# m-schuetz/SimLOD

Measured on NVIDIA H100. Metric: Mpoints/sec octree insertion (16B XYZRGBA), higher is better.
Workload: dtype u32+f32

## Files before the change

### simlod_b200/csrc/construct.cu

```cuda
#include <cooperative_groups.h>
#include <stdint.h>
#include "../../include/simlod_abi.h"
#include "fpmath.cuh"

namespace cg = cooperative_groups;

typedef SimlodPoint Point;
typedef SimlodChunk Chunk;
typedef SimlodNode Node;
typedef SimlodStats Stats;
typedef SimlodUniforms Uniforms;
typedef SimlodHeapHeader Heap;
struct CudaPrint;

#include "construct_layout.cuh"

enum : uint32_t {
    ERR_SPILL_OVERFLOW  = 1u << 0,
    ERR_VOXEL_OVERFLOW  = 1u << 1,
    ERR_DIR_OVERFLOW    = 1u << 2,
    ERR_NODE_OVERFLOW   = 1u << 3,
    ERR_QUEUE_OVERFLOW  = 1u << 4,
    ERR_SPILLNODE_OVERFLOW = 1u << 5,
    ERR_ROW_OVERFLOW    = 1u << 6,
// ... 105 lines not shown
__device__ __forceinline__ bool nested(const Coords& q) {
    return ((((q.pX >> 8) ^ q.X) | ((q.pY >> 8) ^ q.Y) | ((q.pZ >> 8) ^ q.Z)) & 0xfffffu) == 0;
}
__device__ __forceinline__ uint32_t childIndexAt(const Coords& q, uint32_t level) {
    uint32_t sh = SIMLOD_MAX_DEPTH - 1 - level;
    return (((q.X >> sh) & 1u) << 2) | (((q.Y >> sh) & 1u) << 1) | ((q.Z >> sh) & 1u);
}
__device__ __forceinline__ uint32_t cellAt(const Coords& q, uint32_t level) {
    uint32_t sh = SIMLOD_MAX_DEPTH + 1 - level;
    uint32_t cx = (q.pX >> sh) & 127u, cy = (q.pY >> sh) & 127u, cz = (q.pZ >> sh) & 127u;
    return cx | (cy << 7) | (cz << 14);
}

__shared__ uint32_t sh_allocTarget;
__shared__ uint32_t sh_allocSeen;

__device__ __forceinline__ void waitAllocThread(const Ctx& c) {
    const uint32_t target = sh_allocTarget;
    if (target == 0 || *(volatile uint32_t*)&sh_allocSeen) return;
    while ((int32_t)(ldAcquire(&c.ctl()->allocDone) - target) < 0) __nanosleep(64);
    *(volatile uint32_t*)&sh_allocSeen = 1;
}
__device__ __forceinline__ void waitAllocBlock(const Ctx& c) {
    if (sh_allocTarget != 0) {
        if (threadIdx.x == 0) waitAllocThread(c);
        __syncthreads();
    }
}

#ifndef SIMLOD_VOXTAB_SIZE
#define SIMLOD_VOXTAB_SIZE 64
#endif
constexpr uint32_t VOXTAB_SIZE = SIMLOD_VOXTAB_SIZE;
static_assert((VOXTAB_SIZE & (VOXTAB_SIZE - 1)) == 0 && VOXTAB_SIZE <= 128, "table size: a power of two, two tables are flushed by one 256-thread block, the index is packed into 7 bits");
constexpr uint32_t VOXTAB_EMPTY = 0xffffffffu;
__shared__ uint32_t sh_tabKey[VOXTAB_SIZE];
__shared__ uint32_t sh_tabCount[VOXTAB_SIZE];
__shared__ uint32_t sh_tabBase[VOXTAB_SIZE];
__shared__ uint32_t sh_cursor;
__shared__ uint32_t sh_passStart;

__device__ __forceinline__ uint32_t tabHash(uint32_t key) { return (key * 0x9E3779B1u) >> 26; }
__device__ __forceinline__ uint32_t tabFind(const uint32_t* keys, uint32_t key) {
    uint32_t h = tabHash(key);
#pragma unroll 1
    for (uint32_t probe = 0; probe < VOXTAB_SIZE; probe++) {
        uint32_t s = (h + probe) & (VOXTAB_SIZE - 1);
        uint32_t k = keys[s];
        if (k == key) return s;
        if (k == VOXTAB_EMPTY) break;
    }
    return VOXTAB_EMPTY;
}
__device__ __forceinline__ uint32_t tabInsert(uint32_t* keys, uint32_t key) {
    uint32_t h = tabHash(key);
#pragma unroll 1
    for (uint32_t probe = 0; probe < VOXTAB_SIZE; probe++) {
        uint32_t s = (h + probe) & (VOXTAB_SIZE - 1);
        uint32_t k = atomicCAS(&keys[s], VOXTAB_EMPTY, key);
        if (k == VOXTAB_EMPTY || k == key) return s;
    }
    return VOXTAB_EMPTY;
}

__device__ __forceinline__ void voxelPassBegin(const Ctx& c, const Batch& b, bool firstPassOfBatch) {
    if (threadIdx.x < VOXTAB_SIZE) { sh_tabKey[threadIdx.x] = VOXTAB_EMPTY; sh_tabCount[threadIdx.x] = 0; }
    if (threadIdx.x == 0) { sh_cursor = firstPassOfBatch ? 0u : c.blockCursor(b.parity)[blockIdx.x]; sh_passStart = sh_cursor; }
}

__device__ __noinline__ void recordVoxelShared(uint32_t node, uint32_t cell, uint32_t color) {
    const Ctx c;
    const Batch& b = sh_batch;
    waitAllocThread(c);
    Node* nd = &c.nodes()[node];
    uint32_t vslot = atomicAdd(&nd->numVoxels, 1u);
    if (vslot == ldv(&nd->numVoxelsStored)) { uint32_t d = atomicAdd(&b.bc->numDirtyVox, 1u); c.dirtyVox(b.parity)[d] = node; }
    atomicAdd(&b.bc->voxelsCreated, 1u);
    uint32_t e = atomicAdd(&b.bc->numBacklog, 1u);
    if (e < scratch::VOXEL_SHARED) {
        uint64_t at = scratch::VOXEL_CAP - scratch::VOXEL_SHARED + e;
        c.vkey(b.parity)[at] = (uint64_t)cell | ((uint64_t)node << 21) | ((uint64_t)vslot << 41);
        c.vcolor(b.parity)[at] = color;
    } else {
        atomicOr(&c.ctl()->errorFlags, ERR_VOXEL_OVERFLOW);
    }
}

__device__ __forceinline__ void recordVoxel(const Ctx& c, const Batch& b, uint32_t node, uint32_t cell, uint32_t color) {
    const uint32_t active = __activemask();
    const uint32_t leader = __ffs(active) - 1u;
    const uint32_t node0 = __shfl_sync(active, node, leader);
    if (__all_sync(active, node == node0)) {
        const uint32_t n = __popc(active), mine = __popc(active & lanemaskLt());
        uint32_t slot = 0, idx0 = 0, rank0 = 0, fit = 0;
        if (laneId() == leader) {
            slot = tabInsert(sh_tabKey, node0);
            if (slot != VOXTAB_EMPTY) {
                idx0 = atomicAdd(&sh_cursor, n);
                fit = idx0 < c.segCap() ? min(n, c.segCap() - idx0) : 0u;
                if (fit) rank0 = atomicAdd(&sh_tabCount[slot], fit);
            }
        }
        slot = __shfl_sync(active, slot, leader); idx0 = __shfl_sync(active, idx0, leader); rank0 = __shfl_sync(active, rank0, leader); fit = __shfl_sync(active, fit, leader);
        if (mine >= fit) { recordVoxelShared(node, cell, color); return; }
        const uint64_t at = (uint64_t)blockIdx.x * c.segCap() + idx0 + mine;
        c.vkey(b.parity)[at] = (uint64_t)cell | ((uint64_t)slot << 21) | ((uint64_t)(rank0 + mine) << 41);
        c.vcolor(b.parity)[at] = color;
        return;
    }
    uint32_t slot = tabInsert(sh_tabKey, node);
    if (slot == VOXTAB_EMPTY) { recordVoxelShared(node, cell, color); return; }
    uint32_t idx = atomicAdd(&sh_cursor, 1u);
    if (idx >= c.segCap()) { recordVoxelShared(node, cell, color); return; }
    uint32_t rank = atomicAdd(&sh_tabCount[slot], 1u);
    uint64_t at = (uint64_t)blockIdx.x * c.segCap() + idx;
    c.vkey(b.parity)[at] = (uint64_t)cell | ((uint64_t)slot << 21) | ((uint64_t)rank << 41);
    c.vcolor(b.parity)[at] = color;
}

__device__ __forceinline__ void voxelFlushEntry(const Ctx& c, const Batch& b, uint32_t entry) {
    uint32_t node = sh_tabKey[entry], cnt = sh_tabCount[entry];
    if (node != VOXTAB_EMPTY && cnt > 0) {
        Node* nd = &c.nodes()[node];
        uint32_t base = atomicAdd(&nd->numVoxels, cnt);
        if (base == ldv(&nd->numVoxelsStored)) {
            uint32_t d = atomicAdd(&b.bc->numDirtyVox, 1u);
            c.dirtyVox(b.parity)[d] = node;
        }
        sh_tabBase[entry] = base;
    }
}
__device__ __forceinline__ void voxelFlushPatch(const Ctx& c, const Batch& b, bool freshPass) {
    const uint32_t endIdx = min(sh_cursor, c.segCap());
    uint64_t* vkey = c.vkey(b.parity);
    for (uint32_t e = sh_passStart + threadIdx.x; e < endIdx; e += blockDim.x) {
        uint64_t at = (uint64_t)blockIdx.x * c.segCap() + e;
        uint64_t k = vkey[at];
        uint32_t slot = (uint32_t)(k >> 21) & (VOXTAB_SIZE - 1);
        uint32_t rank = (uint32_t)(k >> 41);
        vkey[at] = (k & 0x1fffffull) | ((uint64_t)sh_tabKey[slot] << 21) | ((uint64_t)(sh_tabBase[slot] + rank) << 41);
    }
    if (threadIdx.x == 0) {
        c.blockCursor(b.parity)[blockIdx.x] = endIdx;
        if (endIdx > sh_passStart) {
            atomicAdd(&b.bc->voxelsCreated, endIdx - sh_passStart);
            atomicAdd(reinterpret_cast<unsigned long long*>(&c.ctl()->voxelsTotal), (unsigned long long)(endIdx - sh_passStart));
            atomicAdd(reinterpret_cast<unsigned long long*>(&c.ctl()->voxelsByPass[freshPass ? 0 : 1]), (unsigned long long)(endIdx - sh_passStart));
        }
    }
}

constexpr uint32_t PROVISIONAL = 0x80000000u;
static_assert(scratch::ITEM_CAP < (1u << 24), "block-local ranks must fit 24 bits");
__shared__ uint32_t sh_leafKey[VOXTAB_SIZE];
__shared__ uint32_t sh_leafCount[VOXTAB_SIZE];
__shared__ uint32_t sh_leafBase[VOXTAB_SIZE];
__shared__ uint8_t  sh_leafLevel[VOXTAB_SIZE];
__device__ __forceinline__ uint32_t finalSlot(uint32_t sl) { return (sl & PROVISIONAL) ? sh_leafBase[(sl >> 24) & 127u] + (sl & 0xffffffu) : sl; }
constexpr uint32_t RUNSLOT_CAP = 2048;
__shared__ uint32_t sh_runSlot[RUNSLOT_CAP];
constexpr uint32_t LIST_CAP = 2048;
__shared__ uint32_t sh_listCount;
__shared__ uint32_t sh_listMode;
__shared__ uint32_t sh_blockLegacy;
__shared__ uint8_t  sh_entrySplit[VOXTAB_SIZE];
constexpr uint32_t WL_SPLIT_SHIFT = 22;
constexpr uint32_t WL_ITEM_MASK = (1u << WL_SPLIT_SHIFT) - 1u;
static_assert(scratch::ITEM_CAP <= (1u << WL_SPLIT_SHIFT), "worklist entries keep the item in 22 bits");
__shared__ uint32_t sh_splitNodes[64];
__shared__ SpillInfo sh_splitInfo[64];
__shared__ uint32_t sh_splitGranule[65];
__shared__ uint32_t sh_wlCount, sh_wlBase, sh_wlFill;
__shared__ uint32_t sh_roundLegacy, sh_roundListed;
__device__ __forceinline__ uint32_t blockExclusiveScan(uint32_t v, uint32_t& total) {
    __shared__ uint32_t sh_warpSum[8];
    __shared__ uint32_t sh_total;
    const uint32_t lane = laneId(), warp = threadIdx.x >> 5;
    uint32_t incl = v;
#pragma unroll
    for (int o = 1; o < 32; o <<= 1) { uint32_t t = __shfl_up_sync(0xffffffffu, incl, o); if (lane >= (uint32_t)o) incl += t; }
    __syncthreads();
    if (lane == 31) sh_warpSum[warp] = incl;
    __syncthreads();
    if (threadIdx.x == 0) { uint32_t run = 0; for (int w = 0; w < 8; w++) { uint32_t t = sh_warpSum[w]; sh_warpSum[w] = run; run += t; } sh_total = run; }
    __syncthreads();
    total = sh_total;
    return sh_warpSum[warp] + incl - v;
}

constexpr uint32_t BLOOM_WORDS = 8;
constexpr uint32_t AFFECTED_CAP = 1024;
__shared__ uint32_t sh_runBloom[BLOOM_WORDS];
__shared__ uint32_t sh_affected[AFFECTED_CAP];
__shared__ uint32_t sh_numAffected;
__device__ __forceinline__ uint32_t bloomHash(uint32_t node) { return (node * 0x9E3779B1u) >> 24; }
__device__ __forceinline__ void bloomAdd(uint32_t* bloom, uint32_t node) { uint32_t h = bloomHash(node); atomicOr(&bloom[h >> 5], 1u << (h & 31u)); }

struct Rewalk { uint32_t perRun, runItems, total, spilledBefore; bool listed; };
__device__ __forceinline__ Rewalk rewalkSlice(uint32_t numBatch, uint32_t numSpilled, uint32_t spilledBefore) {
    Rewalk r;
    r.perRun = ((numBatch + gridDim.x - 1) / gridDim.x + 31u) & ~31u;
    r.listed = gridDim.x <= AFFECTED_CAP;
    r.runItems = (r.listed ? sh_numAffected : gridDim.x) * r.perRun;
    r.total = r.runItems + numSpilled;
    r.spilledBefore = spilledBefore;
    return r;
}
__device__ __forceinline__ uint32_t rewalkFirstGranule() { return ((threadIdx.x >> 5) * gridDim.x + blockIdx.x) * 32u; }
__device__ __forceinline__ uint32_t rewalkGranuleStride() { return gridDim.x * blockDim.x; }
__device__ __forceinline__ uint32_t rewalkItem(const Rewalk& r, uint32_t u, uint32_t& run) {
    run = 0xffffffffu;
    if (u >= r.runItems) return (uint32_t)scratch::MAX_BATCH + (u - r.runItems);
    const uint32_t k = u / r.perRun;
    run = r.listed ? sh_affected[k] : k;
    return run * r.perRun + (u - k * r.perRun);
}

__device__ __noinline__ uint32_t countGlobal(uint32_t node, uint32_t level, uint32_t cnt) {
    const Ctx c;
    const Batch& b = sh_batch;
    waitAllocThread(c);
    Node* leaf = &c.nodes()[node];
    uint32_t old = atomicAdd(&leaf->counter, cnt);
    uint32_t stored = ldv(&leaf->numPoints);
    if (old == stored) {
        uint32_t d = atomicAdd(&b.bc->numDirtyLeaves, 1u);
        c.dirtyLeaves(b.parity)[d] = node;
    }
    if (old + cnt > SIMLOD_MAX_POINTS_PER_NODE && atomicCAS(&c.splitState()[node], 0u, 1u) == 0u) {
        uint32_t err = 0;
        const uint32_t childBase = atomicAdd(&c.stats()->numNodes, 8u);
        if ((uint64_t)childBase + 8 > scratch::NODE_CAP) { err = ERR_NODE_OVERFLOW; atomicSub(&c.stats()->numNodes, 8u); }
        uint32_t base = 0;
        if (!err && stored) {
            base = atomicAdd(&b.bc->numSpilled, stored);
            if ((uint64_t)base + stored > scratch::SPILL_CAP) { err = ERR_SPILL_OVERFLOW; atomicSub(&b.bc->numSpilled, stored); atomicSub(&c.stats()->numNodes, 8u); }
        }
        uint32_t s = 0;
        if (!err) {
            s = atomicAdd(&b.bc->numSpillTotal, 1u);
            if (s >= scratch::SPILLNODE_CAP) {
                err = ERR_SPILLNODE_OVERFLOW; atomicSub(&b.bc->numSpillTotal, 1u);
                if (stored) atomicSub(&b.bc->numSpilled, stored);
                atomicSub(&c.stats()->numNodes, 8u);
            }
        }
        if (err) {
            atomicOr(&c.ctl()->errorFlags, err);
            atomicAdd(&c.ctl()->events[3], 1u);
            atomicExch(&c.splitState()[node], 0u);
        } else {
            SpillInfo info;
            info.node = node;
            info.stored = stored;
            info.level = level;
            info.row = c.leafRow()[node];
            info.base = base;
            info.childBase = childBase;
            uint64_t g = c.gridPtr()[node];
            if (g == 0) g = (uint64_t)(c.heapBytes() + atomicAdd(reinterpret_cast<unsigned long long*>(&c.heap()->offset), (unsigned long long)SIMLOD_GRID_STRIDE));
            info.grid = g;
            c.spill()[s] = info;
        }
    }
    return old;
}

struct LeafCache { uint32_t leaf, parent; uint64_t key; };
__device__ __forceinline__ uint64_t leafKey(const Coords& q, uint32_t level) {
    const uint32_t sh = SIMLOD_MAX_DEPTH - level;
    return (uint64_t)((q.X & 0xfffffu) >> sh) | ((uint64_t)((q.Y & 0xfffffu) >> sh) << 20) | ((uint64_t)((q.Z & 0xfffffu) >> sh) << 40);
}

template <bool MIXED_RUNS = false>
__device__ __forceinline__ uint32_t countInto(const Ctx& c, const Batch& b, bool valid, uint32_t node, uint32_t level, uint32_t* bloom, bool forceGlobal) {
    const uint32_t lane = laneId();
    uint32_t slot = 0;
    const uint32_t vmask = __ballot_sync(0xffffffffu, valid);
    if (valid) {
        uint32_t peers = __match_any_sync(vmask, node);
        uint32_t leader = __ffs(peers) - 1;
        uint32_t cnt = __popc(peers);
        uint32_t r = 0;
        if (lane == leader) {
            uint32_t t = forceGlobal ? VOXTAB_EMPTY : tabInsert(sh_leafKey, node);
            if (t != VOXTAB_EMPTY) { r = atomicAdd(&sh_leafCount[t], cnt) | PROVISIONAL | (t << 24); sh_leafLevel[t] = (uint8_t)level; }
            else                 { r = countGlobal(node, level, cnt); sh_blockLegacy = 1; if (!forceGlobal) atomicAdd(&c.ctl()->events[2], 1u); }
            if (bloom) bloomAdd(bloom, node);
        }
        r = __shfl_sync(peers, r, leader);
        slot = r + __popc(peers & lanemaskLt());
        if (MIXED_RUNS) {
            const uint64_t leaderBloom = __shfl_sync(peers, (uint64_t)(uintptr_t)bloom, leader);
            if (bloom && (uint64_t)(uintptr_t)bloom != leaderBloom) bloomAdd(bloom, node);
        }
    }
    return slot;
}

template <bool UNCACHED_GRID, bool DEDUP>
__device__ __forceinline__ void sampleUp(const Ctx& c, const Batch& b, const Coords& q, uint32_t color, uint32_t sNode, uint32_t sLevel, uint32_t stopLevel) {
    const uint32_t lane = laneId();
    const bool exhaustive = !nested(q);
    if (exhaustive) atomicOr(&c.ctl()->errorFlags, ERR_FAR_POINT);
    uint32_t pending = 0;
    uint32_t old0 = 0, old1 = 0, old2 = 0, key0 = 0, key1 = 0, key2 = 0, cel0 = 0, cel1 = 0, cel2 = 0;
    auto settle = [&]() {
        if (pending > 0 && (old0 & (1u << (cel0 & 31u))) == 0) recordVoxel(c, b, key0, cel0, color);
        if (pending > 1 && (old1 & (1u << (cel1 & 31u))) == 0) recordVoxel(c, b, key1, cel1, color);
        if (pending > 2 && (old2 & (1u << (cel2 & 31u))) == 0) recordVoxel(c, b, key2, cel2, color);
        pending = 0;
    };
    const uint64_t* gridPtr = c.gridPtr();
    for (;;) {
        uint64_t g = gridPtr[sNode];
        bool goUp = exhaustive;
        if (g != 0) {
            uint32_t cell = cellAt(q, sLevel);
            uint32_t* word = reinterpret_cast<uint32_t*>(g) + (cell >> 5);
            uint32_t bit = 1u << (cell & 31u);
            uint32_t seen = UNCACHED_GRID ? ldcg(word) : *word;
            if ((seen & bit) == 0) {
                bool mine = true;
                if (DEDUP) {
                    uint32_t active = __activemask();
                    uint32_t peers = __match_any_sync(active, (uint64_t)(uintptr_t)word * 32ull + (cell & 31u));
                    mine = lane == (uint32_t)__ffs(peers) - 1u;
                }
                if (mine) {
                    if (pending == 3) settle();
                    uint32_t old = atomicOr(word, bit);
                    if (pending == 0) { old0 = old; key0 = sNode; cel0 = cell; }
                    else if (pending == 1) { old1 = old; key1 = sNode; cel1 = cell; }
                    else { old2 = old; key2 = sNode; cel2 = cell; }
                    pending++;
                    goUp = true;
                }
            }
        }
        if (!goUp || sLevel <= stopLevel) break;
        sNode = c.parentOf()[sNode];
        sLevel--;
    }
    settle();
}

template <bool SAMPLE, bool COUNT, bool UNCACHED_GRID, bool DEDUP>
__device__ __forceinline__ void walk(const Ctx& c, const Batch& b, LeafCache& cache, bool valid, uint4 pt, uint32_t node, uint32_t level,
                                     uint32_t stopLevel, uint32_t* bloom, bool forceGlobal, uint32_t& leafPacked, uint32_t& slot) {
    Coords q = quantize(c, pt);
    uint32_t parent = VOXTAB_EMPTY;
    if (valid) {
        if (cache.leaf != VOXTAB_EMPTY && leafKey(q, cache.leaf >> 24) == cache.key) {
            node = cache.leaf & 0xffffffu; level = cache.leaf >> 24; parent = cache.parent;
        } else {
            const uint32_t* firstChild = c.firstChild();
#pragma unroll 1
            for (;;) {
                if (level >= SIMLOD_MAX_DEPTH) break;
                uint32_t fc = firstChild[node];
                if (fc == 0) break;
                parent = node;
                node = fc + childIndexAt(q, level);
                level++;
            }
            if (parent == VOXTAB_EMPTY && level > 0) parent = c.parentOf()[node];
            cache.leaf = node | (level << 24); cache.parent = parent; cache.key = leafKey(q, level);
        }
        if (SAMPLE) {
            const uint32_t sNode = level == 0 ? node : parent;
            const uint32_t sLevel = level == 0 ? 0u : level - 1;
            sampleUp<UNCACHED_GRID, DEDUP>(c, b, q, pt.w, sNode, sLevel, stopLevel);
        }
    }
    __syncwarp();

    leafPacked = node | (level << 24);
    if (COUNT) slot = countInto(c, b, valid, node, level, bloom, forceGlobal);
}

#ifndef SIMLOD_REWALK_L2TEST
#define SIMLOD_REWALK_L2TEST 0
#endif
#ifndef SIMLOD_TILE_POINTS
#define SIMLOD_TILE_POINTS 512
#endif
constexpr uint32_t TILE_POINTS = SIMLOD_TILE_POINTS;
static_assert(TILE_POINTS % 256 == 0 && TILE_POINTS >= 256, "a tile is walked in 256-point steps");
__shared__ __align__(128) uint4 sh_tile[2][TILE_POINTS];
__shared__ __align__(8) uint64_t sh_tileBar[2];
__shared__ uint32_t sh_tilePhase[2];

__device__ __forceinline__ void tileBarInit() {
    if (threadIdx.x == 0) {
        uint32_t b0 = (uint32_t)__cvta_generic_to_shared(&sh_tileBar[0]), b1 = (uint32_t)__cvta_generic_to_shared(&sh_tileBar[1]);
        asm volatile("mbarrier.init.shared::cta.b64 [%0], 1;" :: "r"(b0) : "memory");
        asm volatile("mbarrier.init.shared::cta.b64 [%0], 1;" :: "r"(b1) : "memory");
        asm volatile("fence.mbarrier_init.release.cluster;" ::: "memory");
        sh_tilePhase[0] = 0; sh_tilePhase[1] = 0;
    }
    __syncthreads();
}
__device__ __forceinline__ void tileLoad(uint32_t stage, const Point* src, uint32_t numPoints) {
    uint32_t bar = (uint32_t)__cvta_generic_to_shared(&sh_tileBar[stage]);
    uint32_t dst = (uint32_t)__cvta_generic_to_shared(&sh_tile[stage][0]);
    uint32_t bytes = numPoints * 16u;
    asm volatile("mbarrier.arrive.expect_tx.shared::cta.b64 _, [%0], %1;" :: "r"(bar), "r"(bytes) : "memory");
    asm volatile("cp.async.bulk.shared::cluster.global.mbarrier::complete_tx::bytes [%0], [%1], %2, [%3];"
                 :: "r"(dst), "l"(src), "r"(bytes), "r"(bar) : "memory");
}
__device__ __forceinline__ void tileWait(uint32_t stage, uint32_t parity) {
    uint32_t bar = (uint32_t)__cvta_generic_to_shared(&sh_tileBar[stage]);
    uint32_t done;
    do {
        asm volatile("{\n\t.reg .pred p;\n\tmbarrier.try_wait.parity.shared::cta.b64 p, [%1], %2;\n\tselp.u32 %0, 1, 0, p;\n\t}"
                     : "=r"(done) : "r"(bar), "r"(parity) : "memory");
    } while (!done);
}

__device__ __forceinline__ void blockRun(uint32_t numBatch, uint32_t& first, uint32_t& end) {
    const uint32_t perBlock = ((numBatch + gridDim.x - 1) / gridDim.x + 31u) & ~31u;
    first = min(numBatch, blockIdx.x * perBlock);
    end = min(numBatch, first + perBlock);
}

__device__ __forceinline__ void markAffectedRun(const Ctx& c, const Batch& b, uint32_t spillBegin, uint32_t spillEnd) {
    if (threadIdx.x >= 32) return;
    const uint32_t perRun = ((b.size + gridDim.x - 1) / gridDim.x + 31u) & ~31u;
    uint32_t flag = 0;
    if (blockIdx.x * perRun < b.size) {
        const uint32_t* bloom = c.runBloom() + blockIdx.x * BLOOM_WORDS;
        for (uint32_t k = spillBegin + threadIdx.x; k < spillEnd; k += 32) {
            const uint32_t h = bloomHash(c.spill()[k].node);
            flag |= (ldcg(&bloom[h >> 5]) >> (h & 31u)) & 1u;
        }
        flag = __any_sync(0xffffffffu, flag != 0) ? 1u : 0u;
    }
    if (threadIdx.x == 0) c.runFlag()[blockIdx.x] = flag;
}

__device__ __forceinline__ uint32_t* listItem() { return reinterpret_cast<uint32_t*>(&sh_tile[0][0]); }
__device__ __forceinline__ uint32_t* listSlot() { return reinterpret_cast<uint32_t*>(&sh_tile[0][0]) + LIST_CAP; }
static_assert(sizeof(sh_tile) >= LIST_CAP * 8, "the explicit item list must fit the TMA stages");

__device__ void buildWorklist(const Ctx& c, const Batch& b, uint32_t spillBegin, uint32_t spillEnd, uint32_t round) {
    Ctl::Worklist* w = &c.ctl()->wl[b.index % 3u];
    const uint32_t numSplit = spillEnd - spillBegin;
#ifdef SIMLOD_NO_WORKLIST
    if (true) {
#else
    if (numSplit > 64u || sh_blockLegacy != 0) {
#endif
        if (threadIdx.x == 0) atomicExch(&w->legacy, 1u);
        return;
    }
    uint32_t blockFirst, blockEnd;
    blockRun(b.size, blockFirst, blockEnd);
    const uint32_t mode = sh_listMode;
    const uint32_t total = mode == 0 ? blockEnd - blockFirst : min(sh_listCount, LIST_CAP);
    if (threadIdx.x < numSplit) sh_splitNodes[threadIdx.x] = c.spill()[spillBegin + threadIdx.x].node;
    if (threadIdx.x == 0) { sh_wlCount = 0; sh_wlFill = 0; }
    __syncthreads();
    if (threadIdx.x < VOXTAB_SIZE) {
        const uint32_t key = sh_leafKey[threadIdx.x];
        uint32_t f = 0;
        if (key != VOXTAB_EMPTY) for (uint32_t j = 0; j < numSplit; j++) f = key == sh_splitNodes[j] ? j + 1u : f;
        sh_entrySplit[threadIdx.x] = (uint8_t)f;
    }
    __syncthreads();
    const uint32_t* words = mode == 0 ? sh_runSlot : listSlot();
    auto movedAt = [&](uint32_t k) { const uint32_t word = words[k]; return (word & PROVISIONAL) != 0 && sh_entrySplit[(word >> 24) & (VOXTAB_SIZE - 1)] != 0; };
    auto wlSplit = [&](uint32_t word) { return (uint32_t)(sh_entrySplit[(word >> 24) & (VOXTAB_SIZE - 1)] - 1u) << WL_SPLIT_SHIFT; };
    uint32_t cnt = 0;
    for (uint32_t k = threadIdx.x; k < total; k += blockDim.x) cnt += movedAt(k) ? 1u : 0u;
    for (int o = 16; o > 0; o >>= 1) cnt += __shfl_xor_sync(0xffffffffu, cnt, o);
    if (laneId() == 0 && cnt) atomicAdd(&sh_wlCount, cnt);
    __syncthreads();
    if (threadIdx.x == 0) {
        const uint32_t n = sh_wlCount;
        uint32_t base = n ? atomicAdd(&w->cursor[round & 1u], n) : 0u;
        if ((uint64_t)base + n > scratch::WL_CAP) { atomicExch(&w->legacy, 1u); base = 0xffffffffu; }
        sh_wlBase = base;
    }
    __syncthreads();
    const uint32_t base = sh_wlBase;
    if (base == 0xffffffffu || sh_wlCount == 0) return;
    uint32_t* wl = c.worklist();
    const uint32_t* items = listItem();
    for (uint32_t k0 = 0; k0 < total; k0 += blockDim.x) {
        const uint32_t k = k0 + threadIdx.x;
        const bool m = k < total && movedAt(k);
        const uint32_t mask = __ballot_sync(0xffffffffu, m);
        if (mask == 0) continue;
        uint32_t off = 0;
        if (laneId() == 0) off = atomicAdd(&sh_wlFill, (uint32_t)__popc(mask));
        off = __shfl_sync(0xffffffffu, off, 0);
        if (m) wl[base + off + __popc(mask & lanemaskLt())] = (mode == 0 ? blockFirst + k : items[k]) | wlSplit(words[k]);
    }
}

template <bool SAMPLE, bool COUNT, bool FRESH, bool UNCACHED_GRID>
__device__ __forceinline__ void passItems(const Ctx& c, const Batch& b, uint32_t numSpilled, uint32_t spilledBefore, uint32_t round, uint32_t spillBegin = 0, uint32_t spillEnd = 0) {
    uint32_t blockFirst, blockEnd;
    blockRun(b.size, blockFirst, blockEnd);
    LeafCache cache;
    cache.leaf = VOXTAB_EMPTY; cache.parent = VOXTAB_EMPTY; cache.key = 0;

    if (COUNT && threadIdx.x < VOXTAB_SIZE) { sh_leafKey[threadIdx.x] = VOXTAB_EMPTY; sh_leafCount[threadIdx.x] = 0; }
    if (FRESH && COUNT && threadIdx.x < BLOOM_WORDS) sh_runBloom[threadIdx.x] = 0;
    if (FRESH && COUNT && threadIdx.x == 0) { sh_listMode = 0; sh_listCount = 0; sh_blockLegacy = (blockEnd - blockFirst) > RUNSLOT_CAP ? 1u : 0u; }
    if (SAMPLE) voxelPassBegin(c, b, FRESH);
    __syncthreads();

    if (FRESH) {
        const uint32_t runLen = blockEnd - blockFirst;
        const uint32_t numTiles = (runLen + TILE_POINTS - 1) / TILE_POINTS;
        __syncthreads();
        if (threadIdx.x == 0) asm volatile("fence.proxy.async.shared::cta;" ::: "memory");
        if (threadIdx.x == 0 && numTiles > 0) tileLoad(0, b.points + blockFirst, min(TILE_POINTS, runLen));
        for (uint32_t t = 0; t < numTiles; t++) {
            const uint32_t tileFirst = blockFirst + t * TILE_POINTS;
            if (threadIdx.x == 0 && t + 1 < numTiles)
                tileLoad((t + 1) & 1, b.points + tileFirst + TILE_POINTS, min(TILE_POINTS, blockEnd - (tileFirst + TILE_POINTS)));
            tileWait(t & 1, sh_tilePhase[t & 1] ^ ((t >> 1) & 1u));
#pragma unroll 1
            for (uint32_t k = 0; k < TILE_POINTS / 256; k++) {
                const uint32_t idx = k * 256 + threadIdx.x;
                const uint32_t i = tileFirst + idx;
                const bool valid = i < blockEnd;
                uint4 pt = valid ? sh_tile[t & 1][idx] : make_uint4(0, 0, 0, 0);
                uint32_t lp = 0, slot = 0;
                walk<SAMPLE, COUNT, UNCACHED_GRID, true>(c, b, cache, valid, pt, 0, 0, 0, COUNT ? sh_runBloom : nullptr, false, lp, slot);
                if (valid && COUNT) {
                    c.leafOf(b.parity)[i] = lp;
                    if (runLen <= RUNSLOT_CAP) sh_runSlot[i - blockFirst] = slot; else c.slotOf(b.parity)[i] = slot;
                }
            }
            __syncthreads();
        }
        if (threadIdx.x == 0) { sh_tilePhase[0] ^= ((numTiles + 1) >> 1) & 1u; sh_tilePhase[1] ^= (numTiles >> 1) & 1u; }
        if (COUNT && threadIdx.x < BLOOM_WORDS) c.runBloom()[blockIdx.x * BLOOM_WORDS + threadIdx.x] = sh_runBloom[threadIdx.x];
    } else {
        uint32_t* leafOf = c.leafOf(b.parity);
        uint32_t* slotOf = c.slotOf(b.parity);
        if (sh_roundLegacy == 0) {
            const uint32_t listed = min(sh_roundListed, (uint32_t)scratch::WL_CAP);
            const uint32_t perRun = ((b.size + gridDim.x - 1) / gridDim.x + 31u) & ~31u;
            const uint32_t numSplit = spillEnd - spillBegin;
            if (threadIdx.x < numSplit) sh_splitInfo[threadIdx.x] = c.spill()[spillBegin + threadIdx.x];
            if (threadIdx.x == 0) { sh_listCount = 0; sh_listMode = 1; }
            __syncthreads();
            if (threadIdx.x == 0) {
                uint32_t run = 0;
                for (uint32_t k = 0; k < numSplit; k++) { sh_splitGranule[k] = run; run += (sh_splitInfo[k].stored + 31u) / 32u; }
                sh_splitGranule[numSplit] = run;
            }
            __syncthreads();
#if SIMLOD_TIMERS >= 2
            uint64_t tRw = globaltimer();
#define RW_DONE(k) do { __syncthreads(); if (blockIdx.x == 0 && threadIdx.x == 0) { uint64_t _t = globaltimer(); c.ctl()->subNanos[k] += _t - tRw; tRw = _t; } } while (0)
#else
#define RW_DONE(k) do { } while (0)
#endif
            auto reserve = [&](bool valid, bool& forceGlobal) {
                const uint32_t vmask = __ballot_sync(0xffffffffu, valid);
                uint32_t k0 = 0;
                if (laneId() == 0) k0 = atomicAdd(&sh_listCount, (uint32_t)__popc(vmask));
                k0 = __shfl_sync(0xffffffffu, k0, 0);
                forceGlobal = k0 + __popc(vmask) > LIST_CAP;
                if (forceGlobal && laneId() == 0) atomicAdd(&c.ctl()->events[1], 1u);
                return k0 + __popc(vmask & lanemaskLt());
            };
            auto remember = [&](uint32_t i, uint32_t lp, uint32_t slot, uint32_t myk, bool forceGlobal) {
                leafOf[i] = lp;
                if (!forceGlobal) { listItem()[myk] = i; listSlot()[myk] = slot; }
                else {
                    slotOf[i] = slot;
                    if (myk < LIST_CAP) { listItem()[myk] = 0xffffffffu; listSlot()[myk] = 0; }
                }
            };
            RW_DONE(12);
            constexpr uint32_t NO_ITEM = 0xffffffffu;
            auto sampleSplitLeaf = [&](uint64_t grid, const Coords& q, uint32_t color, uint32_t node, uint32_t level) {
                if (!nested(q)) atomicOr(&c.ctl()->errorFlags, ERR_FAR_POINT);
                const uint32_t cell = cellAt(q, level);
                uint32_t* word = reinterpret_cast<uint32_t*>(grid) + (cell >> 5);
                const uint32_t bit = 1u << (cell & 31u);
                const uint32_t seen = (UNCACHED_GRID || SIMLOD_REWALK_L2TEST) ? ldcg(word) : *word;
                if ((seen & bit) == 0 && (atomicOr(word, bit) & bit) == 0) recordVoxel(c, b, node, cell, color);
            };
            {
                const uint32_t share = ((listed + gridDim.x - 1) / gridDim.x + 31u) & ~31u;
                const uint32_t first = min(listed, blockIdx.x * share);
                const uint32_t numListed = min(listed - first, share);
                const uint32_t* wl = c.worklist() + first;
                const uint32_t stride = blockDim.x;
                auto loadEntry = [&](uint32_t bs) { const uint32_t u = bs + laneId(); return u < numListed ? wl[u] : NO_ITEM; };
                auto loadPoint = [&](uint32_t e) {
                    const uint32_t i = e & WL_ITEM_MASK;
                    if (e == NO_ITEM) return make_uint4(0, 0, 0, 0);
                    return i >= scratch::MAX_BATCH ? *reinterpret_cast<const uint4*>(c.spilled() + (i - scratch::MAX_BATCH)) : ldPoint(b.points + i);
                };
                uint32_t base = threadIdx.x & ~31u;
                uint32_t eCur = loadEntry(base), eNext = loadEntry(base + stride);
                uint4 ptCur = loadPoint(eCur);
                for (; base < numListed; base += stride) {
                    const uint4 ptNext = loadPoint(eNext);
                    const uint32_t eNext2 = loadEntry(base + 2u * stride);
                    const uint32_t i = eCur & WL_ITEM_MASK, k = eCur >> WL_SPLIT_SHIFT;
                    const uint4 pt = ptCur;
                    bool valid = eCur != NO_ITEM;
                    const bool spilledItem = valid && i >= scratch::MAX_BATCH;
                    uint32_t node = 0, level = 0, childBase = 0;
                    uint64_t grid = 0;
                    if (valid) {
                        if (k < numSplit) { node = sh_splitInfo[k].node; level = sh_splitInfo[k].level; childBase = sh_splitInfo[k].childBase; grid = sh_splitInfo[k].grid; }
                        else { valid = false; atomicOr(&c.ctl()->errorFlags, ERR_INTERNAL); }
                        valid = valid && level < SIMLOD_MAX_DEPTH;
                    }
                    if (__any_sync(0xffffffffu, valid)) {
                        bool forceGlobal;
                        const uint32_t myk = reserve(valid, forceGlobal);
                        const Coords q = quantize(c, pt);
                        const uint32_t child = childBase + childIndexAt(q, level);
                        if (SAMPLE && valid) sampleSplitLeaf(grid, q, pt.w, node, level);
                        __syncwarp();
                        uint32_t slot = 0;
                        if (COUNT) slot = countInto<true>(c, b, valid, child, level + 1, valid && !spilledItem ? c.runBloom() + (i / perRun) * BLOOM_WORDS : nullptr, forceGlobal);
                        if (valid && COUNT) remember(i, child | ((level + 1) << 24), slot, myk, forceGlobal);
                    }
                    eCur = eNext; ptCur = ptNext; eNext = eNext2;
                }
            }
            RW_DONE(13);
            {
                const uint32_t allGranules = sh_splitGranule[numSplit];
                const uint32_t share = (allGranules + gridDim.x - 1) / gridDim.x;
                const uint32_t gFirst = min(allGranules, blockIdx.x * share);
                const uint32_t numGranules = min(allGranules - gFirst, share);
                const uint32_t gStride = blockDim.x / 32u;
                struct Granule { uint32_t lo, j; bool valid; };
                auto locate = [&](uint32_t g) {
                    Granule r; r.lo = 0; r.j = 0; r.valid = false;
                    if (g < numGranules) {
                        const uint32_t ga = gFirst + g;
                        uint32_t lo = 0, hi = numSplit;
                        while (hi - lo > 1) { const uint32_t mid = (lo + hi) >> 1; if (sh_splitGranule[mid] <= ga) lo = mid; else hi = mid; }
                        const uint32_t within = (ga - sh_splitGranule[lo]) * 32u + laneId();
                        r.lo = lo; r.j = sh_splitInfo[lo].base + within;
                        r.valid = within < sh_splitInfo[lo].stored && sh_splitInfo[lo].level < SIMLOD_MAX_DEPTH;
                    }
                    return r;
                };
                auto loadSpilled = [&](const Granule& gr) { return gr.valid ? *reinterpret_cast<const uint4*>(c.spilled() + gr.j) : make_uint4(0, 0, 0, 0); };
                uint32_t g = threadIdx.x >> 5;
                Granule cur = locate(g);
                uint4 ptCur = loadSpilled(cur);
                for (; g < numGranules; g += gStride) {
                    const Granule next = locate(g + gStride);
                    const uint4 ptNext = loadSpilled(next);
                    const bool valid = cur.valid;
                    if (__any_sync(0xffffffffu, valid)) {
                        const uint32_t node = sh_splitInfo[cur.lo].node, level = sh_splitInfo[cur.lo].level, childBase = sh_splitInfo[cur.lo].childBase;
                        const uint32_t i = (uint32_t)scratch::MAX_BATCH + cur.j;
                        const uint4 pt = ptCur;
                        bool forceGlobal;
                        const uint32_t myk = reserve(valid, forceGlobal);
                        const Coords q = quantize(c, pt);
                        const uint32_t child = childBase + childIndexAt(q, level);
                        if (SAMPLE && valid) sampleSplitLeaf(sh_splitInfo[cur.lo].grid, q, pt.w, node, level);
                        __syncwarp();
                        uint32_t slot = 0;
                        if (COUNT) slot = countInto(c, b, valid, child, level + 1, nullptr, forceGlobal);
                        if (valid && COUNT) remember(i, child | ((level + 1) << 24), slot, myk, forceGlobal);
                    }
                    cur = next; ptCur = ptNext;
                }
            }
            RW_DONE(14);
        } else {
            if (threadIdx.x == 0) sh_blockLegacy = 1;
            if (first_in_grid()) atomicAdd(&c.ctl()->events[0], 1u);
            if (gridDim.x <= AFFECTED_CAP) {
                const uint32_t* flags = c.runFlag();
                uint32_t numAffected = 0;
                for (uint32_t g0 = 0; g0 < gridDim.x; g0 += blockDim.x) {
                    const uint32_t g = g0 + threadIdx.x;
                    const uint32_t flag = g < gridDim.x ? ldcg(&flags[g]) : 0u;
                    uint32_t total = 0;
                    const uint32_t off = blockExclusiveScan(flag, total);
                    if (flag) sh_affected[numAffected + off] = g;
                    numAffected += total;
                }
                if (threadIdx.x == 0) sh_numAffected = numAffected;
                __syncthreads();
            }
            const Rewalk rw = rewalkSlice(b.size, numSpilled, spilledBefore);
            for (uint32_t base = rewalkFirstGranule(); base < rw.total; base += rewalkGranuleStride()) {
                const uint32_t u = base + laneId();
                uint32_t run = 0xffffffffu, i = 0xffffffffu, node = 0, level = 0;
                bool valid = u < rw.total;
                const bool spilledItem = valid && u >= rw.runItems;
                if (valid) { i = rewalkItem(rw, u, run); valid = spilledItem || i < b.size; }
                uint4 pt = make_uint4(0, 0, 0, 0);
                if (spilledItem) pt = *reinterpret_cast<const uint4*>(c.spilled() + (i - scratch::MAX_BATCH));
                if (valid) {
                    uint32_t lp = leafOf[i];
                    node = lp & 0xffffffu; level = lp >> 24;
                    if (!(spilledItem && i - scratch::MAX_BATCH >= rw.spilledBefore)) valid = c.firstChild()[node] != 0 && level < SIMLOD_MAX_DEPTH;
                }
                if (!__any_sync(0xffffffffu, valid)) continue;
                if (valid && !spilledItem) pt = ldPoint(b.points + i);
                uint32_t lp = 0, slot = 0;
                walk<SAMPLE, COUNT, UNCACHED_GRID, false>(c, b, cache, valid, pt, node, level, level, run != 0xffffffffu ? c.runBloom() + run * BLOOM_WORDS : nullptr, false, lp, slot);
                if (valid && COUNT) { leafOf[i] = lp; slotOf[i] = slot; }
            }

        }
    }
    if (FRESH) {
        for (uint32_t base = blockIdx.x * blockDim.x + (threadIdx.x & ~31u); base < numSpilled; base += gridDim.x * blockDim.x) {
            uint32_t j = base + laneId();
            bool valid = j < numSpilled;
            uint4 pt = make_uint4(0, 0, 0, 0);
            if (valid) pt = *reinterpret_cast<const uint4*>(c.spilled() + j);
            uint32_t lp = 0, slot = 0;
            walk<SAMPLE, COUNT, UNCACHED_GRID, true>(c, b, cache, valid, pt, 0, 0, 0, nullptr, false, lp, slot);
        }
    }
    __syncthreads();
}

template <bool SAMPLE, bool COUNT, bool FRESH>
__device__ __forceinline__ void passFlush(const Ctx& c, const Batch& b, uint32_t numSpilled, uint32_t spilledBefore) {
    if (COUNT && threadIdx.x < VOXTAB_SIZE) {
        uint32_t leaf = sh_leafKey[threadIdx.x], cnt = sh_leafCount[threadIdx.x];
        if (leaf != VOXTAB_EMPTY && cnt > 0) sh_leafBase[threadIdx.x] = countGlobal(leaf, sh_leafLevel[threadIdx.x], cnt);
    } else if (SAMPLE && threadIdx.x >= 128 && threadIdx.x < 128 + VOXTAB_SIZE) {
        voxelFlushEntry(c, b, threadIdx.x - 128);
    }
    __syncthreads();
    if (SAMPLE) voxelFlushPatch(c, b, FRESH);
    if (COUNT) {
        uint32_t* slotOf = c.slotOf(b.parity);
        if (FRESH) {
            uint32_t blockFirst, blockEnd;
            blockRun(b.size, blockFirst, blockEnd);
            if (blockEnd - blockFirst <= RUNSLOT_CAP) {
                for (uint32_t i = blockFirst + threadIdx.x; i < blockEnd; i += blockDim.x) slotOf[i] = finalSlot(sh_runSlot[i - blockFirst]);
            } else {
                for (uint32_t i = blockFirst + threadIdx.x; i < blockEnd; i += blockDim.x) { uint32_t sl = slotOf[i]; if (sl & PROVISIONAL) slotOf[i] = finalSlot(sl); }
            }
        } else if (sh_roundLegacy == 0) {
            const uint32_t n = min(sh_listCount, LIST_CAP);
            const uint32_t* li = listItem();
            const uint32_t* ls = listSlot();
            for (uint32_t k = threadIdx.x; k < n; k += blockDim.x) if (li[k] != 0xffffffffu) slotOf[li[k]] = finalSlot(ls[k]);
        } else {
            const Rewalk rw = rewalkSlice(b.size, numSpilled, spilledBefore);
            for (uint32_t base = rewalkFirstGranule(); base < rw.total; base += rewalkGranuleStride()) {
                const uint32_t u = base + laneId();
                if (u >= rw.total) continue;
                uint32_t run;
                const uint32_t i = rewalkItem(rw, u, run);
                if (u < rw.runItems && i >= b.size) continue;
                uint32_t sl = slotOf[i];
                if (sl & PROVISIONAL) slotOf[i] = finalSlot(sl);
            }
        }
    }
    __syncthreads();
}

constexpr uint32_t SPLIT_COPY_PARTS = 256, SPLIT_CLEAR_PARTS = 32, SPLIT_PARTS = SPLIT_COPY_PARTS + SPLIT_CLEAR_PARTS + 1;

__device__ __noinline__ void splitRound(uint32_t begin, uint32_t end) {
    const Ctx c;
    const Batch& b = sh_batch;
    const uint32_t numWarps = (gridDim.x * blockDim.x) >> 5;
    const uint32_t warp = (threadIdx.x >> 5) * gridDim.x + blockIdx.x;
    const uint32_t lane = laneId();
    const uint32_t numItems = (end - begin) * SPLIT_PARTS;
    uint32_t* leafOf = c.leafOf(b.parity);
    for (uint32_t item = warp; item < numItems; item += numWarps) {
        const SpillInfo info = c.spill()[begin + item / SPLIT_PARTS];
        const uint32_t part = item % SPLIT_PARTS;
        const uint32_t numChunks = (info.stored + SIMLOD_POINTS_PER_CHUNK - 1) / SIMLOD_POINTS_PER_CHUNK;
        if (part < SPLIT_COPY_PARTS) {
            const uint32_t k = part >> 2, quarter = part & 3u;
            if (k >= numChunks || info.row == 0) continue;
            const Chunk* chunk = reinterpret_cast<const Chunk*>(c.rows()[(uint64_t)(info.row - 1) * scratch::ROW_SLOTS + k]);
            const uint32_t inChunk = min((uint32_t)SIMLOD_POINTS_PER_CHUNK, info.stored - k * SIMLOD_POINTS_PER_CHUNK);
            const uint32_t first = quarter * 256u;
            const uint32_t n = inChunk > first ? min(256u, inChunk - first) : 0u;
            const uint32_t tag = info.node | (info.level << 24);
            const uint4* src = reinterpret_cast<const uint4*>(&chunk->points[first]);
            const uint32_t dst = info.base + k * SIMLOD_POINTS_PER_CHUNK + first;
#pragma unroll 1
            for (uint32_t h = 0; h < 256u; h += 128u) {
                uint4 v[4];
#pragma unroll
                for (int u = 0; u < 4; u++) if (h + lane + 32u * u < n) v[u] = src[h + lane + 32u * u];
#pragma unroll
                for (int u = 0; u < 4; u++) if (h + lane + 32u * u < n) {
                    *reinterpret_cast<uint4*>(c.spilled() + dst + h + lane + 32u * u) = v[u];
                    leafOf[scratch::MAX_BATCH + dst + h + lane + 32u * u] = tag;
                }
            }
        } else if (part < SPLIT_COPY_PARTS + SPLIT_CLEAR_PARTS) {
            constexpr uint32_t PER = SIMLOD_GRID_WORDS / 4 / SPLIT_CLEAR_PARTS;
            uint4* g = reinterpret_cast<uint4*>(info.grid) + (uint64_t)(part - SPLIT_COPY_PARTS) * PER;
#pragma unroll 4
            for (uint32_t i = lane; i < PER; i += 32) g[i] = make_uint4(0, 0, 0, 0);
        } else {
            Node* parent = &c.nodes()[info.node];
            const uint32_t pX = parent->X, pY = parent->Y, pZ = parent->Z;
            if (lane < 8) {
                Node* child = &c.nodes()[info.childBase + lane];
                uint64_t* raw = reinterpret_cast<uint64_t*>(child);
#pragma unroll
                for (int w = 0; w < 19; w++) raw[w] = 0;
                child->level = info.level + 1;
                child->X = 2 * pX + ((lane >> 2) & 1);
                child->Y = 2 * pY + ((lane >> 1) & 1);
                child->Z = 2 * pZ + (lane & 1);
                for (int k = 0; k < 20; k++) child->name[k] = parent->name[k];
                reinterpret_cast<uint8_t*>(child)[offsetof(Node, name) + info.level + 1] = (uint8_t)('0' + lane);
                child->isLeaf = 1;
                parent->children[lane] = child;
                c.firstChild()[info.childBase + lane] = 0;
                c.parentOf()[info.childBase + lane] = info.node;
                c.gridPtr()[info.childBase + lane] = 0;
                c.leafRow()[info.childBase + lane] = 0;
                c.splitState()[info.childBase + lane] = 0;
            }
            if (numChunks > 0 && info.row != 0) {
                uint64_t a0 = 0;
                if (lane == 0) a0 = atomicAdd(reinterpret_cast<unsigned long long*>(&c.stats()->numAllocatedChunks), (unsigned long long)(0ull - numChunks));
                a0 = __shfl_sync(0xffffffffu, a0, 0);
                for (uint32_t k = lane; k < numChunks && k < scratch::ROW_SLOTS; k += 32) {
                    Chunk* chunk = reinterpret_cast<Chunk*>(c.rows()[(uint64_t)(info.row - 1) * scratch::ROW_SLOTS + k]);
                    chunk->next = nullptr;
                    uint64_t qi = a0 - 1 - k;
                    if (qi < scratch::QUEUE_CAP) c.chunkQueue()[qi] = (uint64_t)chunk;
                    else atomicOr(&c.ctl()->errorFlags, ERR_QUEUE_OVERFLOW);
                }
            }
            __syncwarp();
            if (lane == 0) {
                if (info.row != 0) {
                    uint32_t f = atomicAdd(&c.ctl()->rowFreeCount, 1u);
                    c.rowFree()[f] = info.row;
                    c.leafRow()[info.node] = 0;
                }
                parent->numPoints = 0;
                parent->points = nullptr;
                parent->grid = reinterpret_cast<SimlodOccupancyGrid*>(info.grid);
                c.gridPtr()[info.node] = info.grid;
                c.firstChild()[info.node] = info.childBase;
            }
        }
    }
}

__device__ __noinline__ void allocateChunks() {
    const Ctx c;
    const Batch& b = sh_loop.pending;
    const uint32_t FULL = 0xffffffffu;
    const uint32_t lane = laneId();
    const uint32_t numWarps = (gridDim.x * blockDim.x) >> 5;
    const uint32_t warp = (threadIdx.x >> 5) * gridDim.x + blockIdx.x;
    const uint32_t numDirtyLeaves = ldv(&b.bc->numDirtyLeaves);
    const uint32_t numDirtyVox = ldv(&b.bc->numDirtyVox);
    const uint64_t poolSize = ldv(&c.stats()->chunkPoolSize);
    const uint32_t* dirtyLeaves = c.dirtyLeaves(b.parity);
    const uint32_t* dirtyVox = c.dirtyVox(b.parity);

    for (uint32_t d = warp; d < numDirtyLeaves; d += numWarps) {
        const uint32_t n = dirtyLeaves[d];
        if (c.firstChild()[n] != 0) continue;
        Node* node = &c.nodes()[n];
        const uint32_t cnt = node->counter, have = node->numPoints;
        if (cnt <= have) continue;
        const uint32_t existing = (have + SIMLOD_POINTS_PER_CHUNK - 1) / SIMLOD_POINTS_PER_CHUNK;
        uint32_t required = (cnt + SIMLOD_POINTS_PER_CHUNK - 1) / SIMLOD_POINTS_PER_CHUNK;
        if (required > scratch::ROW_SLOTS) { if (lane == 0) atomicOr(&c.ctl()->errorFlags, ERR_ROW_OVERFLOW); required = scratch::ROW_SLOTS; }
        const uint32_t needed = required > existing ? required - existing : 0;
        if (needed > 0) {
            uint64_t a0 = 0, freshOff = 0;
            uint32_t row = 0;
            if (lane == 0) {
                a0 = atomicAdd(reinterpret_cast<unsigned long long*>(&c.stats()->numAllocatedChunks), (unsigned long long)needed);
                const uint64_t firstFresh = a0 > poolSize ? a0 : poolSize;
                const uint64_t numFresh = a0 + needed > firstFresh ? a0 + needed - firstFresh : 0;
                if (numFresh) {
                    freshOff = atomicAdd(reinterpret_cast<unsigned long long*>(&c.heap()->offset), (unsigned long long)(numFresh * SIMLOD_CHUNK_STRIDE));
                    atomicAdd(reinterpret_cast<unsigned long long*>(&c.ctl()->freshBytes), (unsigned long long)(numFresh * SIMLOD_CHUNK_STRIDE));
                }
                row = c.leafRow()[n];
                if (row == 0) {
                    uint32_t f = atomicSub(&c.ctl()->rowFreeCount, 1u);
                    if (f >= 1 && f <= scratch::ROW_CAP) {
                        row = c.rowFree()[f - 1];
                    } else {
                        atomicAdd(&c.ctl()->rowFreeCount, 1u);
                        uint32_t r = atomicAdd(&c.ctl()->rowBump, 1u);
                        if (r >= scratch::ROW_CAP) { atomicOr(&c.ctl()->errorFlags, ERR_ROW_OVERFLOW); row = 0; }
                        else row = r + 1;
                    }
                    c.leafRow()[n] = row;
// ... 492 lines not shown
```

Baseline: 5961.

## Count split-node children in direct-indexed shared slots instead of hash table

During refinement rounds after node splits, points are now counted into a direct-indexed shared array keyed by (split index, octant) rather than inserting child node IDs into the shared leaf hash table. The one-split path derives warp peer groups from three ballots instead of match_any, and the flush and worklist construction use the new child slot encoding. This is meant to remove hash-table insertion, probing and overflow-to-global fallbacks for children. In exchange it adds a separate slot encoding with an 11-bit rank limit and more shared memory.

```diff
diff --git a/simlod_b200/csrc/construct.cu b/simlod_b200/csrc/construct.cu
--- a/simlod_b200/csrc/construct.cu
+++ b/simlod_b200/csrc/construct.cu
@@ -281,6 +281,14 @@
 
 constexpr uint32_t PROVISIONAL = 0x80000000u;
 static_assert(scratch::ITEM_CAP < (1u << 24), "block-local ranks must fit 24 bits");
+constexpr uint32_t CHILD_RANK_BITS = 11;
+constexpr uint32_t CHILD_SLOTS = 64 * 8;
+__shared__ uint32_t sh_childCount[CHILD_SLOTS];
+__shared__ uint8_t  sh_childSplit[CHILD_SLOTS];
+__shared__ uint32_t sh_roundSplits;
+__device__ __forceinline__ uint32_t childWord(uint32_t e, uint32_t rank) { return PROVISIONAL | (e << CHILD_RANK_BITS) | rank; }
+__device__ __forceinline__ uint32_t childOf(uint32_t sl) { return (sl >> CHILD_RANK_BITS) & (CHILD_SLOTS - 1u); }
+__device__ __forceinline__ uint32_t finalChildSlot(uint32_t sl) { return (sl & PROVISIONAL) ? sh_childCount[childOf(sl)] + (sl & ((1u << CHILD_RANK_BITS) - 1u)) : sl; }
 __shared__ uint32_t sh_leafKey[VOXTAB_SIZE];
 __shared__ uint32_t sh_leafCount[VOXTAB_SIZE];
 __shared__ uint32_t sh_leafBase[VOXTAB_SIZE];
@@ -289,6 +297,7 @@
 constexpr uint32_t RUNSLOT_CAP = 2048;
 __shared__ uint32_t sh_runSlot[RUNSLOT_CAP];
 constexpr uint32_t LIST_CAP = 2048;
+static_assert(LIST_CAP <= (1u << CHILD_RANK_BITS), "a child's block-local ranks must fit its slot word");
 __shared__ uint32_t sh_listCount;
 __shared__ uint32_t sh_listMode;
 __shared__ uint32_t sh_blockLegacy;
@@ -422,6 +431,35 @@
         if (MIXED_RUNS) {
             const uint64_t leaderBloom = __shfl_sync(peers, (uint64_t)(uintptr_t)bloom, leader);
             if (bloom && (uint64_t)(uintptr_t)bloom != leaderBloom) bloomAdd(bloom, node);
+        }
+    }
+    return slot;
+}
+
+template <bool ONE_SPLIT, bool MIXED_RUNS>
+__device__ __forceinline__ uint32_t countChild(bool valid, uint32_t e, uint32_t child, uint32_t level, uint32_t* bloom, bool forceGlobal) {
+    const uint32_t lane = laneId();
+    uint32_t slot = 0;
+    const uint32_t vmask = __ballot_sync(0xffffffffu, valid);
+    uint32_t peers = 0;
+    if (ONE_SPLIT) {
+        const uint32_t b0 = __ballot_sync(0xffffffffu, e & 1u), b1 = __ballot_sync(0xffffffffu, e & 2u), b2 = __ballot_sync(0xffffffffu, e & 4u);
+        peers = vmask & ((e & 1u) ? b0 : ~b0) & ((e & 2u) ? b1 : ~b1) & ((e & 4u) ? b2 : ~b2);
+    }
+    if (valid) {
+        if (!ONE_SPLIT) peers = __match_any_sync(vmask, e);
+        const uint32_t leader = __ffs(peers) - 1;
+        uint32_t r = 0;
+        if (lane == leader) {
+            if (!forceGlobal) r = childWord(e, atomicAdd(&sh_childCount[e], (uint32_t)__popc(peers)));
+            else              { r = countGlobal(child, level, __popc(peers)); sh_blockLegacy = 1; }
+            if (bloom) bloomAdd(bloom, child);
+        }
+        r = __shfl_sync(peers, r, leader);
+        slot = r + __popc(peers & lanemaskLt());
+        if (MIXED_RUNS) {
+            const uint64_t leaderBloom = __shfl_sync(peers, (uint64_t)(uintptr_t)bloom, leader);
+            if (bloom && (uint64_t)(uintptr_t)bloom != leaderBloom) bloomAdd(bloom, child);
         }
     }
     return slot;
@@ -587,19 +625,35 @@
     blockRun(b.size, blockFirst, blockEnd);
     const uint32_t mode = sh_listMode;
     const uint32_t total = mode == 0 ? blockEnd - blockFirst : min(sh_listCount, LIST_CAP);
-    if (threadIdx.x < numSplit) sh_splitNodes[threadIdx.x] = c.spill()[spillBegin + threadIdx.x].node;
     if (threadIdx.x == 0) { sh_wlCount = 0; sh_wlFill = 0; }
-    __syncthreads();
-    if (threadIdx.x < VOXTAB_SIZE) {
-        const uint32_t key = sh_leafKey[threadIdx.x];
-        uint32_t f = 0;
-        if (key != VOXTAB_EMPTY) for (uint32_t j = 0; j < numSplit; j++) f = key == sh_splitNodes[j] ? j + 1u : f;
-        sh_entrySplit[threadIdx.x] = (uint8_t)f;
+    if (mode == 0) {
+        if (threadIdx.x < numSplit) sh_splitNodes[threadIdx.x] = c.spill()[spillBegin + threadIdx.x].node;
+        __syncthreads();
+        if (threadIdx.x < VOXTAB_SIZE) {
+            const uint32_t key = sh_leafKey[threadIdx.x];
+            uint32_t f = 0;
+            if (key != VOXTAB_EMPTY) for (uint32_t j = 0; j < numSplit; j++) f = key == sh_splitNodes[j] ? j + 1u : f;
+            sh_entrySplit[threadIdx.x] = (uint8_t)f;
+        }
+    } else {
+        for (uint32_t e = threadIdx.x; e < CHILD_SLOTS; e += blockDim.x) sh_childSplit[e] = 0;
+        __syncthreads();
+        if (threadIdx.x < numSplit) {
+            const uint32_t node = c.spill()[spillBegin + threadIdx.x].node;
+            for (uint32_t k = 0; k < sh_roundSplits; k++) {
+                const uint32_t o = node - sh_splitInfo[k].childBase;
+                if (o < 8u) sh_childSplit[k * 8u + o] = (uint8_t)(threadIdx.x + 1u);
+            }
+        }
     }
     __syncthreads();
     const uint32_t* words = mode == 0 ? sh_runSlot : listSlot();
-    auto movedAt = [&](uint32_t k) { const uint32_t word = words[k]; return (word & PROVISIONAL) != 0 && sh_entrySplit[(word >> 24) & (VOXTAB_SIZE - 1)] != 0; };
-    auto wlSplit = [&](uint32_t word) { return (uint32_t)(sh_entrySplit[(word >> 24) & (VOXTAB_SIZE - 1)] - 1u) << WL_SPLIT_SHIFT; };
+    auto splitOf = [&](uint32_t word) -> uint32_t {
+        if ((word & PROVISIONAL) == 0) return 0u;
+        return mode == 0 ? sh_entrySplit[(word >> 24) & (VOXTAB_SIZE - 1)] : sh_childSplit[childOf(word)];
+    };
+    auto movedAt = [&](uint32_t k) { return splitOf(words[k]) != 0; };
+    auto wlSplit = [&](uint32_t word) { return (splitOf(word) - 1u) << WL_SPLIT_SHIFT; };
     uint32_t cnt = 0;
     for (uint32_t k = threadIdx.x; k < total; k += blockDim.x) cnt += movedAt(k) ? 1u : 0u;
     for (int o = 16; o > 0; o >>= 1) cnt += __shfl_xor_sync(0xffffffffu, cnt, o);
@@ -677,7 +731,8 @@
             const uint32_t perRun = ((b.size + gridDim.x - 1) / gridDim.x + 31u) & ~31u;
             const uint32_t numSplit = spillEnd - spillBegin;
             if (threadIdx.x < numSplit) sh_splitInfo[threadIdx.x] = c.spill()[spillBegin + threadIdx.x];
-            if (threadIdx.x == 0) { sh_listCount = 0; sh_listMode = 1; }
+            for (uint32_t e = threadIdx.x; e < CHILD_SLOTS; e += blockDim.x) sh_childCount[e] = 0;
+            if (threadIdx.x == 0) { sh_listCount = 0; sh_listMode = 1; sh_roundSplits = numSplit; }
             __syncthreads();
             if (threadIdx.x == 0) {
                 uint32_t run = 0;
@@ -751,11 +806,15 @@
                         bool forceGlobal;
                         const uint32_t myk = reserve(valid, forceGlobal);
                         const Coords q = quantize(c, pt);
-                        const uint32_t child = childBase + childIndexAt(q, level);
+                        const uint32_t octant = childIndexAt(q, level);
+                        const uint32_t child = childBase + octant;
                         if (SAMPLE && valid) sampleSplitLeaf(grid, q, pt.w, node, level);
                         __syncwarp();
                         uint32_t slot = 0;
-                        if (COUNT) slot = countInto<true>(c, b, valid, child, level + 1, valid && !spilledItem ? c.runBloom() + (i / perRun) * BLOOM_WORDS : nullptr, forceGlobal);
+                        if (COUNT) {
+                            uint32_t* bloom = valid && !spilledItem ? c.runBloom() + (i / perRun) * BLOOM_WORDS : nullptr;
+                            slot = countChild<false, true>(valid, k * 8u + octant, child, level + 1, bloom, forceGlobal);
+                        }
                         if (valid && COUNT) remember(i, child | ((level + 1) << 24), slot, myk, forceGlobal);
                     }
                     eCur = eNext; ptCur = ptNext; eNext = eNext2;
@@ -796,11 +855,12 @@
                         bool forceGlobal;
                         const uint32_t myk = reserve(valid, forceGlobal);
                         const Coords q = quantize(c, pt);
-                        const uint32_t child = childBase + childIndexAt(q, level);
+                        const uint32_t octant = childIndexAt(q, level);
+                        const uint32_t child = childBase + octant;
                         if (SAMPLE && valid) sampleSplitLeaf(sh_splitInfo[cur.lo].grid, q, pt.w, node, level);
                         __syncwarp();
                         uint32_t slot = 0;
-                        if (COUNT) slot = countInto(c, b, valid, child, level + 1, nullptr, forceGlobal);
+                        if (COUNT) slot = countChild<true, false>(valid, cur.lo * 8u + octant, child, level + 1, nullptr, forceGlobal);
                         if (valid && COUNT) remember(i, child | ((level + 1) << 24), slot, myk, forceGlobal);
                     }
                     cur = next; ptCur = ptNext;
@@ -862,7 +922,13 @@
 
 template <bool SAMPLE, bool COUNT, bool FRESH>
 __device__ __forceinline__ void passFlush(const Ctx& c, const Batch& b, uint32_t numSpilled, uint32_t spilledBefore) {
-    if (COUNT && threadIdx.x < VOXTAB_SIZE) {
+    if (COUNT && !FRESH && sh_roundLegacy == 0) {
+        for (uint32_t e = threadIdx.x; e < sh_roundSplits * 8u; e += blockDim.x) {
+            const uint32_t cnt = sh_childCount[e];
+            if (cnt > 0) sh_childCount[e] = countGlobal(sh_splitInfo[e >> 3].childBase + (e & 7u), sh_splitInfo[e >> 3].level + 1u, cnt);
+        }
+        if (SAMPLE && threadIdx.x >= 128 && threadIdx.x < 128 + VOXTAB_SIZE) voxelFlushEntry(c, b, threadIdx.x - 128);
+    } else if (COUNT && threadIdx.x < VOXTAB_SIZE) {
         uint32_t leaf = sh_leafKey[threadIdx.x], cnt = sh_leafCount[threadIdx.x];
         if (leaf != VOXTAB_EMPTY && cnt > 0) sh_leafBase[threadIdx.x] = countGlobal(leaf, sh_leafLevel[threadIdx.x], cnt);
     } else if (SAMPLE && threadIdx.x >= 128 && threadIdx.x < 128 + VOXTAB_SIZE) {
@@ -884,7 +950,7 @@
             const uint32_t n = min(sh_listCount, LIST_CAP);
             const uint32_t* li = listItem();
             const uint32_t* ls = listSlot();
-            for (uint32_t k = threadIdx.x; k < n; k += blockDim.x) if (li[k] != 0xffffffffu) slotOf[li[k]] = finalSlot(ls[k]);
+            for (uint32_t k = threadIdx.x; k < n; k += blockDim.x) if (li[k] != 0xffffffffu) slotOf[li[k]] = finalChildSlot(ls[k]);
         } else {
             const Rewalk rw = rewalkSlice(b.size, numSpilled, spilledBefore);
             for (uint32_t base = rewalkFirstGranule(); base < rw.total; base += rewalkGranuleStride()) {
```

After: 6386, median of 6. 7.1% higher.
